# microsoft/SEAL-Embedded

Measured on AMD Instinct MI355X. Metric: CKKS ciphertexts/s (batched encode+encrypt), higher is better.
Workload: dtype u32; 1 GPU; C2: n=4096, 3x30-bit RNS primes, symmetric encode+encrypt, batch=65536 per GPU; n=4096, nprimes=3, mode=sym, batch_per_gpu=65536, global_batch=65536, parallelism=batch-sharded x1, bytes_per_unit=106624

## Files before the change

include/seal_embedded_amd.h:

```cpp
#ifndef SEAL_EMBEDDED_AMD_H
#define SEAL_EMBEDDED_AMD_H

#include <stdbool.h>
#include <stddef.h>
#include <stdint.h>
#include <sys/types.h>

#ifdef __cplusplus
typedef double _Complex se_complex;
#else
#include <complex.h>
typedef double complex se_complex;
#endif

#ifdef __cplusplus
extern "C" {
#endif

#define SE_SUCCESS 0
#define SE_ERR_NO_MEMORY -12
#define SE_ERR_INVALD_ARGUMENT -22
#define SE_ERR_UNKNOWN -1000
#define SE_ERR_MINIMUM -9999
#define SE_ERR_NO_DEVICE -19
// ... 175 lines not shown
int se_amd_write_ciphertext_text(const char *path, int append, const float *values, size_t vlen,
                                 const uint32_t *c0, const uint32_t *c1, size_t n, size_t np);
int se_amd_save_secret_key_file(const char *dir, size_t n, const uint8_t *sk_packed);
int se_amd_save_public_key_files(const char *dir, size_t n, size_t np, const uint32_t *q,
                                 const uint32_t *pk0, const uint32_t *pk1);

enum
{
    SE_AMD_STAGE_CBD = 0,
    SE_AMD_STAGE_UNIFORM = 1,
    SE_AMD_STAGE_TERNARY = 2,
    SE_AMD_STAGE_ENCODE_ENCRYPT = 3,
    SE_AMD_STAGE_ENCODE_RNS = 4,
    SE_AMD_STAGE_NTT_FUSE = 5,
    SE_AMD_STAGE_COUNT = 6
};
int se_amd_set_profiling(se_amd_ctx *ctx, int enabled);
int se_amd_stage_ms(se_amd_ctx *ctx, float *ms ,
                    uint64_t *launches , int reset);
int se_amd_host_tables(size_t degree, size_t nprimes, uint32_t *q, uint32_t *const_ratio,
                       double *scale, uint16_t *index_map, double *ifft_w, uint32_t *ntt_rw,
                       uint32_t *intt_rw);
int se_amd_ifft_table_sha256(se_amd_ctx *ctx, char out_hex[65]);
int se_amd_set_reject_list_capacity(se_amd_ctx *ctx, uint32_t cap);
int se_amd_set_speculation_capacity(se_amd_ctx *ctx, uint32_t cap);
int se_amd_set_host_chunk(se_amd_ctx *ctx, size_t ciphertexts);
int se_amd_reserve(se_amd_ctx *ctx, size_t B);
int se_amd_set_debug_flags(se_amd_ctx *ctx, uint32_t flags);
int se_amd_set_pipeline(se_amd_ctx *ctx, int overlap, int split);
int se_amd_set_asym_chunks(se_amd_ctx *ctx, size_t chunks);
const char *se_amd_last_error(void);
const char *se_amd_version(void);

#ifdef __cplusplus
}
#endif

#include "seal_embedded_amd_lower.h"

#endif
```

seal-embedded_amd/__init__.py:

```python
import ctypes as C
import os
import subprocess

HERE = os.path.dirname(os.path.abspath(__file__))
LIB_PATH = os.path.join(HERE, "lib", "libseal_embedded_amd.so")
CSRC = os.path.join(HERE, "csrc")
INCLUDE = os.path.join(os.path.dirname(HERE), "include", "seal_embedded_amd.h")

STAGES = ("cbd", "uniform", "ternary", "encode_encrypt", "encode_rns", "ntt_fuse")

SE_SUCCESS = 0


class SealEmbeddedAmdError(RuntimeError):
    pass


TESTHOOKS_LIB_DIR = os.path.join(HERE, "lib", "testhooks")


def build_library(jobs=8, verbose=False):
    cmd = ["make", "-C", CSRC, f"-j{jobs}", "all", "testhooks"]
    if not verbose:
        cmd.insert(1, "-s")
# ... 3 lines not shown

_lib = None

EXPORTED_SYMBOLS = (
    "se_setup_custom", "se_setup", "se_setup_default", "se_encrypt_seeded", "se_encrypt",
    "se_cleanup", "se_encrypt_batch",
    "se_amd_create", "se_amd_destroy", "se_amd_degree", "se_amd_nprimes", "se_amd_scale",
    "se_amd_moduli", "se_amd_index_map", "se_amd_set_secret_key", "se_amd_set_public_key",
    "se_amd_load_keys_from_dir", "se_amd_gen_public_key", "se_amd_gen_keys_batch", "se_amd_encrypt_sym_device", "se_amd_encrypt_asym_device", "se_amd_encrypt_sym_seeded_device",
    "se_amd_expand_c1_device",
    "se_amd_encode_ntt_device", "se_amd_encrypt_sym_host", "se_amd_encrypt_asym_host",
    "se_amd_encode_device", "se_amd_ntt_device", "se_amd_intt_device", "se_amd_decrypt_decode_device", "se_amd_prng_blocks_device",
    "se_amd_sample_uniform_device", "se_amd_sample_ternary_device", "se_amd_sample_cbd_device",
    "se_amd_pack_ternary_host", "se_amd_word_ops_device", "se_amd_pack_seal_ciphertext_host", "se_amd_format_poly_text",
    "se_amd_format_values_text", "se_amd_write_ciphertext_text", "se_amd_save_secret_key_file",
    "se_amd_save_public_key_files", "se_amd_set_profiling", "se_amd_stage_ms",
    "se_amd_group_create", "se_amd_group_destroy", "se_amd_group_size", "se_amd_group_ctx", "se_amd_group_device",
    "se_amd_group_partition", "se_amd_group_set_secret_key", "se_amd_group_set_public_key", "se_amd_group_reserve",
    "se_amd_encrypt_sym_multi_device", "se_amd_encrypt_asym_multi_device", "se_amd_encode_ntt_multi_device",
    "se_amd_set_reject_list_capacity", "se_amd_set_speculation_capacity", "se_amd_set_host_chunk", "se_amd_host_tables", "se_amd_ifft_table_sha256", "se_amd_reserve", "se_amd_set_debug_flags", "se_amd_set_pipeline", "se_amd_set_asym_chunks", "se_amd_last_error", "se_amd_version",
    "se_amd_set_secret_keyring", "se_amd_set_public_keyring", "se_amd_encrypt_sym_keyed_device",
    "se_amd_encrypt_asym_keyed_device", "se_amd_decrypt_decode_keyed_device",
    "se_amd_decrypt_full_device", "se_amd_decrypt_full_keyed_device", "se_amd_crt_constants",
)


def lib():
    global _lib
    if _lib is not None:
        return _lib
    if not os.path.exists(LIB_PATH):
        raise SealEmbeddedAmdError(
            f"{LIB_PATH} is missing: run __graft_entry__.build() (hipcc --offload-arch=gfx950). "
            "There is no CPU fallback.")
    L = C.CDLL(LIB_PATH)
    vp, sz, i32, u32 = C.c_void_p, C.c_size_t, C.c_int, C.c_uint32
    L.se_amd_last_error.restype = C.c_char_p
    L.se_amd_version.restype = C.c_char_p
    L.se_amd_create.argtypes = [C.POINTER(vp), sz, sz, i32]
    L.se_amd_destroy.argtypes = [vp]
    L.se_amd_destroy.restype = None
    L.se_amd_degree.argtypes = [vp]
    L.se_amd_degree.restype = sz
    L.se_amd_nprimes.argtypes = [vp]
    L.se_amd_nprimes.restype = sz
    L.se_amd_scale.argtypes = [vp]
# ... 19 lines not shown
    L.se_amd_prng_blocks_device.argtypes = [vp, vp, vp, vp, sz, sz, vp]
    L.se_amd_sample_uniform_device.argtypes = [vp, vp, vp, sz, vp, vp, vp]
    L.se_amd_sample_ternary_device.argtypes = [vp, vp, sz, vp, vp, vp]
    L.se_amd_sample_cbd_device.argtypes = [vp, vp, vp, sz, sz, vp, vp]
    L.se_amd_word_ops_device.argtypes = [vp, sz, i32, vp, vp, vp, vp, sz, vp]
    L.se_amd_pack_ternary_host.argtypes = [vp, sz, vp]
    L.se_amd_pack_ternary_host.restype = None
    L.se_amd_pack_seal_ciphertext_host.argtypes = [vp, vp, sz, sz, vp]
    L.se_amd_pack_seal_ciphertext_host.restype = None
    L.se_amd_format_poly_text.argtypes = [C.c_char_p, vp, sz, vp, sz]
    L.se_amd_format_poly_text.restype = sz
    L.se_amd_format_values_text.argtypes = [C.c_char_p, vp, sz, vp, sz]
    L.se_amd_format_values_text.restype = sz
    L.se_amd_write_ciphertext_text.argtypes = [C.c_char_p, i32, vp, sz, vp, vp, sz, sz]
    L.se_amd_save_secret_key_file.argtypes = [C.c_char_p, sz, vp]
    L.se_amd_save_public_key_files.argtypes = [C.c_char_p, sz, sz, vp, vp, vp]
    L.se_amd_set_profiling.argtypes = [vp, i32]
    L.se_amd_stage_ms.argtypes = [vp, vp, vp, i32]
    L.se_amd_set_reject_list_capacity.argtypes = [vp, u32]
    L.se_amd_set_speculation_capacity.argtypes = [vp, u32]
    L.se_amd_set_host_chunk.argtypes = [vp, sz]
    L.se_amd_host_tables.argtypes = [sz, sz, vp, vp, vp, vp, vp, vp, vp]
    L.se_amd_ifft_table_sha256.argtypes = [vp, C.c_char_p]
    L.se_amd_reserve.argtypes = [vp, sz]
    L.se_amd_set_debug_flags.argtypes = [vp, u32]
    L.se_amd_set_pipeline.argtypes = [vp, i32, i32]
    L.se_amd_set_asym_chunks.argtypes = [vp, sz]
    L.se_amd_set_secret_keyring.argtypes = [vp, sz, vp]
    L.se_amd_set_public_keyring.argtypes = [vp, sz, vp, vp]
    L.se_amd_encrypt_sym_keyed_device.argtypes = [vp, vp, sz, vp, vp, vp, vp, vp, vp, vp, vp, vp]
    L.se_amd_encrypt_asym_keyed_device.argtypes = [vp, vp, sz, vp, vp, vp, vp, vp, vp, vp, vp]
    L.se_amd_decrypt_decode_keyed_device.argtypes = [vp, vp, vp, sz, vp, sz, vp, vp, vp, vp]
    L.se_amd_decrypt_full_device.argtypes = [vp, vp, vp, sz, vp, vp, vp, vp, vp]
    L.se_amd_decrypt_full_keyed_device.argtypes = [vp, vp, vp, sz, vp, vp, vp, vp, vp, vp]
    L.se_amd_crt_constants.argtypes = [sz, sz, vp, vp]
    _lib = L
    return L


def _check(rc, what):
    if rc < 0:
        msg = lib().se_amd_last_error().decode(errors="replace")
        raise SealEmbeddedAmdError(f"{what} failed with code {rc}: {msg}")
    return rc


# ... 124 lines not shown
        except Exception:
            pass

    def scale(self):
        return float(self.L.se_amd_scale(self.h))

    def moduli(self):
        import numpy as np
        q = np.zeros(self.np, dtype=np.uint32)
        _check(self.L.se_amd_moduli(self.h, _ptr(q)), "se_amd_moduli")
        return [int(x) for x in q]

    def index_map(self):
        import numpy as np
        m = np.zeros(self.n, dtype=np.uint16)
        _check(self.L.se_amd_index_map(self.h, _ptr(m)), "se_amd_index_map")
        return m

    def ifft_table_sha256(self):
        buf = C.create_string_buffer(65)
        _check(self.L.se_amd_ifft_table_sha256(self.h, buf), "se_amd_ifft_table_sha256")
        return buf.value.decode()

    def set_secret_key(self, sk_packed):
        import numpy as np
        sk = np.ascontiguousarray(sk_packed, dtype=np.uint8)
        assert sk.size == self.n // 4
        _check(self.L.se_amd_set_secret_key(self.h, _ptr(sk)), "se_amd_set_secret_key")

    def set_public_key(self, pk0, pk1):
        import numpy as np
        pk0 = np.ascontiguousarray(pk0, dtype=np.uint32)
        pk1 = np.ascontiguousarray(pk1, dtype=np.uint32)
        assert pk0.size == self.np * self.n == pk1.size
        _check(self.L.se_amd_set_public_key(self.h, _ptr(pk0), _ptr(pk1)), "se_amd_set_public_key")

    def gen_public_key(self, sk_packed, pk_seed, ep_seed):
        import numpy as np
        sk = np.ascontiguousarray(sk_packed, dtype=np.uint8)
        s1 = np.frombuffer(bytes(pk_seed), dtype=np.uint8).copy()
        s2 = np.frombuffer(bytes(ep_seed), dtype=np.uint8).copy()
        pk0 = np.zeros((self.np, self.n), dtype=np.uint32)
        pk1 = np.zeros_like(pk0)
        _check(self.L.se_amd_gen_public_key(self.h, _ptr(sk), _ptr(s1), _ptr(s2), _ptr(pk0),
                                            _ptr(pk1)), "se_amd_gen_public_key")
        return pk0, pk1
# ... 227 lines not shown
```

seal-embedded_amd/csrc/kernels/encode_encrypt.hip:

```cpp
#include <hip/hip_runtime.h>

#include <algorithm>

#include "../se_types.h"
#include "kernel_args.h"
#include "transform.cuh"

namespace seamd {

__device__ __forceinline__ void load16(uint32_t (&v)[16], const uint32_t *p)
{
    const uint4 *p4 = reinterpret_cast<const uint4 *>(p);
#pragma unroll
    for (int i = 0; i < 4; i++)
    {
        uint4 w      = p4[i];
        v[4 * i]     = w.x;
        v[4 * i + 1] = w.y;
        v[4 * i + 2] = w.z;
        v[4 * i + 3] = w.w;
    }
}

__device__ __forceinline__ void store16(uint32_t *p, const uint32_t (&v)[16])
// ... 203 lines not shown
    }
    wg = __ockl_wgred_or_i32((ok ? 0 : kWgOverflow) | (small ? 0 : kWgNotSmall) | (nonfinite ? kWgNonfinite : 0));
    if constexpr (sizeof(MT) == 4)
    {
        small = !(wg & kWgNotSmall);
        if (status && t == 0 && small) status[b] = 1;
    }
    else
    {
        const bool declined = !BRANCH_EXACT && (wg & kWgNonfinite);
        if (status && t == 0 && !declined) status[b] = (wg & kWgOverflow) ? 0 : 1;
    }
}

template <int MODE>
constexpr int enc_quad_stride()
{
    return MODE == kModeAsym ? 28 : 20;
}

constexpr int kWgRisky          = 8;
constexpr double kHalfDelta     = 3.0e-14 * 1.001;
constexpr size_t kPairParkWords = 5120;

template <int LOGN, int MODE, bool GENERAL, bool PAIR, typename MT>
__device__ __forceinline__ void encrypt_tail(const DevParams &P, const DevTables &T, const EncArgs &A,
                                             const size_t b, unsigned char *smem, MT (&m)[16], const bool small)
{
    const int t = thread_index<GENERAL>();
    using G            = XformGeom<LOGN>;
    constexpr bool ASYM3 = LOGN <= 12;
    constexpr int N    = G::N;
    constexpr int CTOP = LOGN - 4;
    uint32_t *lds32 = reinterpret_cast<uint32_t *>(smem);

    const int np   = P.nprimes;

    if constexpr (MODE == kModeSym)
    {
#pragma unroll
        for (int e = 0; e < 16; e++) m[e] += A.err[b * N + (e << CTOP) + t];
    }
    else if constexpr (MODE == kModeAsym)
    {
#pragma unroll
        for (int e = 0; e < 16; e++) m[e] += A.err[b * 2 * N + (e << CTOP) + t];
// ... 121 lines not shown
                st_poly<QUADS>(A.c1 + pb, out, tg);
            }
            reduce_signed16(m, x, q, crh, crl, small);
            ntt_tiles<LOGN>(x, RW, q, lds32, t);
#pragma unroll
            for (int e = 0; e < 16; e++) x[e] = canon4(x[e], q, two_q);
            to_quads(x);
            if (A.ntt_pte) st_poly<QUADS>(A.ntt_pte + pb, x, tg);
            park_load();
            {
                uint32_t w[16], wp[16], out[16];
                ld_pairs<QUADS>(w, wp, T.pk0 + kb, tg);
#pragma unroll
                for (int e = 0; e < 16; e++)
                {
                    uint32_t pr = csub(mul_shoup_lazy(uh[e], w[e], wp[e], q), q);
                    out[e]      = csub(pr + x[e], q);
                }
                st_poly<QUADS>(A.c0 + pb, out, tg);
            }
        }
        else
        {
            uint32_t a_pre[16];
            if constexpr (MODE == kModeSym && QUADS) ld_poly<QUADS>(a_pre, A.c1 + pb, tg);
            reduce_signed16(m, x, q, crh, crl, small);
            ntt_tiles<LOGN>(x, RW, q, lds32, t);
            if constexpr (MODE != kModeSym)
            {
#pragma unroll
                for (int e = 0; e < 16; e++) x[e] = canon4(x[e], q, two_q);
            }
            to_quads(x);
            if (A.ntt_pte)
            {
                uint32_t cx[16];
#pragma unroll
                for (int e = 0; e < 16; e++) cx[e] = canon4(x[e], q, two_q);
                st_poly<QUADS>(A.ntt_pte + pb, cx, tg);
            }
            if constexpr (MODE == kModeSym)
            {
                uint32_t a[16], w[16], wp[16], out[16];
                if constexpr (QUADS)
                {
#pragma unroll
                    for (int e = 0; e < 16; e++) a[e] = a_pre[e];
                }
                else
                    ld_poly<QUADS>(a, A.c1 + pb, tg);
// ... 82 lines not shown
    for (int p = 0; p < 2; p++)
    {
        const float s = nf[p].x + nf[p].y;
        nonfinite[p]  = s != s;
    }
    __syncthreads();
    const float ss_all[2] = {(part[0] + part[2]) + (part[4] + part[6]), (part[1] + part[3]) + (part[5] + part[7])};
    double re[16], im[16];
    {
        const int Tl    = t & 127;
        const float *my = sv + (t >> 7) * (N / 2);
        const uint4 *mp = reinterpret_cast<const uint4 *>(T.gather_map);
        uint4 m0 = mp[Tl], m1 = mp[TH + Tl];
        uint32_t packed[8] = {m0.x, m0.y, m0.z, m0.w, m1.x, m1.y, m1.z, m1.w};
#pragma unroll
        for (int e = 0; e < 16; e++)
        {
            uint32_t idx = (packed[e >> 1] >> (16 * (e & 1))) & 0xFFFFu;
            re[e]        = (double)my[idx];
            im[e]        = 0.0;
        }
    }
    __syncthreads();
    ifft_pair_real_half<LOGN>(re, im, T.ifft_w, plane, t);

    int flags = 0;
#pragma unroll
    for (int p = 0; p < 2; p++)
    {
        const double delta = kHalfDelta * P.n_inv * sqrt(2.0 * (double)N * (double)ss_all[p]);
        double amax = 0.0;
        bool risky  = false;
#pragma unroll
        for (int e = 0; e < 16; e++)
        {
            const double x = e < 8 ? re[8 * p + e] : im[8 * p + e - 8];
            const double v = __dmul_rn(x, P.n_inv);
            const double a = fabs(v);
            const double g = __dsub_rn(a, trunc(a));
            risky          = risky || (fabs(__dsub_rn(g, 0.5)) < delta);
            const double r = round_half_away(v);
            amax           = fmax(amax, fabs(r));
            if (p == 0) mA[e] = (int32_t)r; else mB[e] = (int32_t)r;
        }
        const bool sm = amax < P.small_bound && !nonfinite[p];
        flags |= ((sm ? 0 : kWgNotSmall) | (nonfinite[p] ? kWgNonfinite : 0) | (risky ? kWgRisky : 0)) << (8 * p);
    }
// ... 736 lines not shown
    return hipGetLastError();
}

hipError_t launch_key_sanitize(const uint32_t *raw, uint32_t *idx, uint32_t *bad, size_t K, size_t B, hipStream_t st)
{
    if (B == 0) return hipSuccess;
    if (K == 0 || K > 0xFFFFFFFFull) return hipErrorInvalidValue;
    hipError_t e = hipMemsetAsync(bad, 0, sizeof(uint32_t), st);
    if (e != hipSuccess) return e;
    hipLaunchKernelGGL(k_key_sanitize, dim3((unsigned)((B + 255) / 256)), dim3(256), 0, st, raw, idx, bad,
                       (uint32_t)K, B);
    return hipGetLastError();
}

hipError_t launch_key_reject(const DevParams &P, const KeyRejectArgs &A, size_t B, hipStream_t st)
{
    if (B == 0) return hipSuccess;
    const unsigned grid = (unsigned)std::min<size_t>(B, (size_t)4 * (P.num_cus ? P.num_cus : 256u));
    hipLaunchKernelGGL(k_key_reject, dim3(grid), dim3(256), 0, st, A);
    return hipGetLastError();
}

template <int LOGN, int MODE>
static hipError_t launch_enc_mode(const DevParams &P, const DevTables &T, const EncArgs &A, size_t B,
                                  hipStream_t st, const KeyRing *ring)
{
    using G             = XformGeom<LOGN>;
    const size_t planes = (size_t)G::SLOTS * sizeof(double);
    const size_t quads  = (size_t)(G::N / 16) * enc_quad_stride<MODE>() * sizeof(uint32_t);
    size_t shmem_fast = planes, shmem_gen = planes;
    if (LOGN <= 12)
    {
        const size_t ntt_planes = (size_t)(MODE == kModeAsym ? 3 : 1) * G::SLOTS * sizeof(uint32_t);
        shmem_fast = MODE == kModeAsym ? std::max(planes, std::max(ntt_planes, quads)) : std::max(planes, ntt_planes + quads);
        shmem_gen  = MODE == kModeAsym ? std::max(planes, ntt_planes) : std::max(planes, ntt_planes + quads);
    }
    hipError_t e = hipMemsetAsync(A.general, 0, sizeof(uint32_t), st);
    if (e != hipSuccess) return e;
    EncArgs Af = A;
    Af.count   = B;
    if (enc_pairs<LOGN, MODE>()) shmem_fast = std::max(shmem_fast, (kPairParkWords + (size_t)G::N) * sizeof(uint32_t));
    const unsigned grid_fast = (unsigned)(enc_pairs<LOGN, MODE>() ? (B + 1) / 2 : B);
    const unsigned cus  = P.num_cus ? P.num_cus : 256u;
    const unsigned grid = (unsigned)std::min<size_t>(B, (size_t)4 * cus);
    if constexpr (MODE != kModeEncodeOnly)
    {
        if (ring)
        {
            (void)hipFuncSetAttribute((const void *)k_encode_encrypt_keyed<LOGN, MODE>,
                                      hipFuncAttributeMaxDynamicSharedMemorySize, (int)shmem_fast);
            hipLaunchKernelGGL((k_encode_encrypt_keyed<LOGN, MODE>), dim3(grid_fast), dim3(G::THREADS), shmem_fast, st,
                               P, T, Af, *ring);
            e = hipGetLastError();
            if (e != hipSuccess) return e;
            (void)hipFuncSetAttribute((const void *)k_encode_encrypt_general_keyed<LOGN, MODE>,
                                      hipFuncAttributeMaxDynamicSharedMemorySize, (int)shmem_gen);
            hipLaunchKernelGGL((k_encode_encrypt_general_keyed<LOGN, MODE>), dim3(grid), dim3(G::THREADS), shmem_gen,
                               st, P, T, A, *ring);
            return hipGetLastError();
        }
    }
    (void)hipFuncSetAttribute((const void *)k_encode_encrypt<LOGN, MODE>,
                              hipFuncAttributeMaxDynamicSharedMemorySize, (int)shmem_fast);
    hipLaunchKernelGGL((k_encode_encrypt<LOGN, MODE>), dim3(grid_fast), dim3(G::THREADS), shmem_fast, st, P, T,
// ... 13 lines not shown
{
    if (!A.general) return hipErrorInvalidValue;
    switch (mode)
    {
        case kModeSym: return launch_enc_mode<LOGN, kModeSym>(P, T, A, B, st, ring);
        case kModeAsym: return launch_enc_mode<LOGN, kModeAsym>(P, T, A, B, st, ring);
        default:
            if (ring) return hipErrorInvalidValue;
            return launch_enc_mode<LOGN, kModeEncodeOnly>(P, T, A, B, st, nullptr);
    }
}

hipError_t launch_encode_encrypt(const DevParams &P, const DevTables &T, const EncArgs &A, int mode,
                                 size_t B, hipStream_t st, const KeyRing *ring)
{
    if (B == 0) return hipSuccess;
    switch (P.logn)
    {
        case 10: return launch_enc<10>(P, T, A, mode, B, st, ring);
        case 11: return launch_enc<11>(P, T, A, mode, B, st, ring);
        case 12: return launch_enc<12>(P, T, A, mode, B, st, ring);
        case 13: return launch_enc<13>(P, T, A, mode, B, st, ring);
        case 14: return launch_enc<14>(P, T, A, mode, B, st, ring);
        default: return hipErrorInvalidValue;
    }
}

template <int LOGN, bool ADD_ERR>
static hipError_t launch_enc_rns_e(const DevParams &P, const DevTables &T, const EncArgs &A, size_t B,
                                   hipStream_t st)
{
    using G      = XformGeom<LOGN>;
    size_t shmem = (size_t)G::SLOTS * sizeof(double);
    if (!A.general) return hipErrorInvalidValue;
    hipError_t e = hipMemsetAsync(A.general, 0, sizeof(uint32_t), st);
    if (e != hipSuccess) return e;
    (void)hipFuncSetAttribute((const void *)k_encode_rns<LOGN, ADD_ERR>,
                              hipFuncAttributeMaxDynamicSharedMemorySize, (int)shmem);
    hipLaunchKernelGGL((k_encode_rns<LOGN, ADD_ERR>), dim3((unsigned)B), dim3(G::THREADS), shmem, st, P, T, A);
    e = hipGetLastError();
    if (e != hipSuccess) return e;
    const unsigned cus  = P.num_cus ? P.num_cus : 256u;
    const unsigned grid = (unsigned)std::min<size_t>(B, (size_t)cus);
    (void)hipFuncSetAttribute((const void *)k_encode_rns_general<LOGN, ADD_ERR>,
                              hipFuncAttributeMaxDynamicSharedMemorySize, (int)shmem);
    hipLaunchKernelGGL((k_encode_rns_general<LOGN, ADD_ERR>), dim3(grid), dim3(G::THREADS), shmem, st, P, T, A);
// ... 108 lines not shown
```

seal-embedded_amd/csrc/kernels/kernel_args.h:

```cpp
#pragma once
#include <hip/hip_runtime.h>
#include <stddef.h>
#include <stdint.h>

#include "../se_types.h"

namespace seamd {

struct EncArgs
{
    const float *values;
    const int8_t *err;
    const int8_t *ucodes;
    uint32_t *c0;
    uint32_t *c1;
    uint32_t *ntt_pte;
    int64_t *pte;
    uint8_t *status;
    uint32_t *general;
    uint8_t *compact;
    size_t count;
};
struct UniformArgs
{
// ... 28 lines not shown
};
struct TernaryArgs
{
    const uint8_t *seeds;
    int8_t *codes;
    uint64_t *ctr_out;
    uint32_t n;
    uint32_t B;
    const uint64_t *ctr_in;
    uint32_t num_cus;
    uint32_t debug_flags;
};

struct KeyRing
{
    const uint32_t *k0;
    const uint32_t *k1;
    const uint32_t *idx;
    size_t stride;
};

hipError_t launch_encode_encrypt(const DevParams &, const DevTables &, const EncArgs &, int mode,
                                 size_t B, hipStream_t, const KeyRing *ring = nullptr);
hipError_t launch_encode_rns(const DevParams &, const DevTables &, const EncArgs &, bool add_err,
                             size_t B, hipStream_t);
hipError_t launch_ntt_fuse(const DevParams &, const DevTables &, const EncArgs &, int mode, int j,
                           size_t B, hipStream_t, const KeyRing *ring = nullptr);
hipError_t launch_decrypt_decode(const DevParams &, const DevTables &, const uint32_t *c0,
                                 const uint32_t *c1, uint32_t in_primes, int j, uint32_t *dec_ntt,
                                 uint32_t *pt, float *values, size_t B, hipStream_t,
                                 const KeyRing *ring = nullptr);
struct FullArgs
{
    const uint32_t *c0;
    const uint32_t *c1;
    int64_t *pte;
    float *values;
    double *values_f64;
    uint8_t *status;
};
hipError_t launch_decrypt_full(const DevParams &, const DevTables &, const CrtParams &, const FullArgs &, size_t B,
                               hipStream_t, const KeyRing *ring = nullptr);
hipError_t launch_ring_secret_ntt(const DevParams &, const DevTables &, int j, const uint8_t *packed, uint32_t *ring,
                                  size_t K, hipStream_t);
hipError_t launch_ring_pairs(const DevParams &, const uint32_t *vals, uint32_t *pairs, size_t K, hipStream_t);
hipError_t launch_key_sanitize(const uint32_t *raw, uint32_t *idx, uint32_t *bad, size_t K, size_t B, hipStream_t);
// ... 85 lines not shown
```

seal-embedded_amd/csrc/kernels/transform.cuh:

```cuda
#pragma once
#include <hip/hip_runtime.h>
#include <stdint.h>

#include <type_traits>

#include "modarith.cuh"

namespace seamd {

template <int BEGIN, int END, typename F>
__device__ __forceinline__ void static_for(F &&f)
{
    if constexpr (BEGIN < END)
    {
        f(std::integral_constant<int, BEGIN>{});
        static_for<BEGIN + 1, END>(f);
    }
}

template <int C>
__device__ __forceinline__ int tile_index(int t, int e)
{
    return ((t >> C) << (C + 4)) | (e << C) | (t & ((1 << C) - 1));
}

template <int CA, int CB>
__host__ __device__ constexpr int lds_slot(int k)
{
    constexpr int lo = CA < CB ? CA : CB, hi = CA < CB ? CB : CA;
    if constexpr (hi <= 4)
        return k + (k >> 4);
    else if constexpr (lo >= 5)
        return k;
    else
        return k + ((k >> 5) << 1);
}

template <int LOGN>
struct XformGeom
{
    static constexpr int N       = 1 << LOGN;
    static constexpr int THREADS = N / 16;
    static constexpr int PASSES  = (LOGN + 3) / 4;
    static constexpr int SLOTS   = N + N / 16;
    static constexpr int ifft_c(int p) { return (4 * p < LOGN - 4) ? 4 * p : LOGN - 4; }
    static constexpr int ntt_c(int p) { return (LOGN - 4 - 4 * p > 0) ? LOGN - 4 - 4 * p : 0; }
};

template <int C_FROM, int C_TO, typename T>
__device__ __forceinline__ void redeal(T (&v)[16], T *lds, int t)
{
    T *wr = lds + lds_slot<C_FROM, C_TO>(tile_index<C_FROM>(t, 0));
    static_for<0, 16>([&](auto ec) {
        constexpr int e = decltype(ec)::value;
        wr[lds_slot<C_FROM, C_TO>(e << C_FROM)] = v[e];
    });
    __syncthreads();
    const T *rd = lds + lds_slot<C_FROM, C_TO>(tile_index<C_TO>(t, 0));
    static_for<0, 16>([&](auto ec) {
        constexpr int e = decltype(ec)::value;
        v[e] = rd[lds_slot<C_FROM, C_TO>(e << C_TO)];
    });
    __syncthreads();
}

template <int STRIDE>
__device__ __forceinline__ void tile_to_quads(uint32_t (&x)[16], uint32_t *lds_region, int t)
{
    static_assert(STRIDE % 4 == 0 && STRIDE >= 16, "rows stay 16-byte aligned");
    const int lane = t & 63;
// ... 57 lines not shown
        if (dev_isnan(d)) d = dev_copysign(0.0, d);
        recalc = true;
    }
    if (recalc)
    {
        const double inf = __longlong_as_double(0x7FF0000000000000ll);
        x = __dmul_rn(inf, __dsub_rn(__dmul_rn(a, c), __dmul_rn(b, d)));
        y = __dmul_rn(inf, __dadd_rn(__dmul_rn(a, d), __dmul_rn(b, c)));
    }
}

template <bool EXACT>
__device__ __forceinline__ void cmul_annexg(double a, double b, double c, double d, double &x, double &y)
{
    const double ac = __dmul_rn(a, c), bd = __dmul_rn(b, d), ad = __dmul_rn(a, d), bc = __dmul_rn(b, c);
    x = __dsub_rn(ac, bd);
    y = __dadd_rn(ad, bc);
    if constexpr (EXACT)
    {
        if (dev_isnan(x) && dev_isnan(y)) cmul_recover(a, b, c, d, ac, bd, ad, bc, x, y);
    }
}

template <int LOGN, int C, int B_LO, int B_HI, bool EXACT = false>
__device__ __forceinline__ void ifft_pass(double (&re)[16], double (&im)[16],
                                          const double *__restrict__ W, int t)
{
    constexpr int N = 1 << LOGN;
    const int thi   = (C + 4 >= LOGN) ? 0 : (t >> C);
    static_for<B_LO, B_HI>([&](auto bc) {
        constexpr int b      = decltype(bc)::value;
        constexpr int h      = N >> (C + b + 1);
        constexpr int groups = 1 << (3 - b);
        static_for<0, groups>([&](auto gc) {
            constexpr int g = decltype(gc)::value;
            const int idx   = (C == 0) ? N + ((8 >> b) - 1 + g) * (N / 16) + t : h + ((thi << (3 - b)) | g);
            const double2 w = *reinterpret_cast<const double2 *>(W + 2 * idx);
            static_for<0, (1 << b)>([&](auto rc) {
                constexpr int e0 = (g << (b + 1)) | decltype(rc)::value;
                constexpr int e1 = e0 | (1 << b);
                double ar = __dsub_rn(re[e0], re[e1]);
                double ai = __dsub_rn(im[e0], im[e1]);
                re[e0]    = __dadd_rn(re[e0], re[e1]);
                im[e0]    = __dadd_rn(im[e0], im[e1]);
                cmul_annexg<EXACT>(ar, ai, w.x, w.y, re[e1], im[e1]);
            });
        });
    });
}

template <int LOGN>
__device__ __forceinline__ void ifft_pass0_real(double (&re)[16], double (&im)[16],
                                                const double *__restrict__ W, int t)
{
    constexpr int N = 1 << LOGN;
    static_for<0, 4>([&](auto bc) {
        constexpr int b      = decltype(bc)::value;
        constexpr int groups = 1 << (3 - b);
        static_for<0, groups>([&](auto gc) {
// ... 38 lines not shown
    redeal<0, 4>(im, plane, t);
    ifft_pass<LOGN, 4, 0, 4, EXACT>(re, im, W, t);
    if constexpr (LOGN <= 12)
    {
        constexpr int C2 = G::ifft_c(2);
        redeal<4, C2>(re, plane, t);
        redeal<4, C2>(im, plane, t);
        ifft_pass<LOGN, C2, 8 - C2, 4, EXACT>(re, im, W, t);
    }
    else
    {
        redeal<4, 8>(re, plane, t);
        redeal<4, 8>(im, plane, t);
        ifft_pass<LOGN, 8, 0, 4, EXACT>(re, im, W, t);
        constexpr int C3 = G::ifft_c(3);
        redeal<8, C3>(re, plane, t);
        redeal<8, C3>(im, plane, t);
        ifft_pass<LOGN, C3, 12 - C3, 4, EXACT>(re, im, W, t);
    }
}

template <int LOGN>
__device__ __forceinline__ void ifft_pair_real_half(double (&re)[16], double (&im)[16], const double *__restrict__ W,
                                                    double *plane, int t)
{
    static_assert(LOGN == 12, "four waves: two per plaintext in the register passes");
    using G             = XformGeom<LOGN>;
    constexpr int N     = 1 << LOGN;
    constexpr int HALF  = G::SLOTS / 2;
    static_assert(lds_slot<0, 4>(N / 2 - 1) < HALF && lds_slot<4, 8>(N / 2 - 1) < HALF, "a plaintext's lower half fits its region");
    const int T   = t & 127;
    double *mine  = plane + (t >> 7) * HALF;
    ifft_pass0_real<LOGN>(re, im, W, T);
    auto exchange_0_4 = [&](double (&v)[16]) {
        double *wr = mine + lds_slot<0, 4>(tile_index<0>(T, 0));
        static_for<0, 16>([&](auto ec) {
            constexpr int e = decltype(ec)::value;
            wr[lds_slot<0, 4>(e << 0)] = v[e];
        });
        __syncthreads();
        const double *rd = mine + lds_slot<0, 4>(tile_index<4>(T, 0));
        static_for<0, 16>([&](auto ec) {
            constexpr int e = decltype(ec)::value;
            v[e] = rd[lds_slot<0, 4>(e << 4)];
        });
        __syncthreads();
    };
    exchange_0_4(re);
    exchange_0_4(im);
    ifft_pass<LOGN, 4, 0, 4>(re, im, W, T);
    auto exchange_4_8 = [&](double (&v)[16]) {
        double *wr = mine + lds_slot<4, 8>(tile_index<4>(T, 0));
        static_for<0, 16>([&](auto ec) {
            constexpr int e = decltype(ec)::value;
            wr[lds_slot<4, 8>(e << 4)] = v[e];
        });
        __syncthreads();
        const double *rd = plane + lds_slot<4, 8>(tile_index<8>(t, 0));
        static_for<0, 8>([&](auto ec) {
            constexpr int e = decltype(ec)::value;
            v[e]     = rd[lds_slot<4, 8>(e << 8)];
            v[8 + e] = rd[HALF + lds_slot<4, 8>(e << 8)];
        });
        __syncthreads();
    };
    exchange_4_8(re);
    exchange_4_8(im);
    static_for<0, 3>([&](auto bc) {
        constexpr int b = decltype(bc)::value;
        constexpr int h = N >> (8 + b + 1);
        static_for<0, (4 >> b)>([&](auto gc) {
            constexpr int g = decltype(gc)::value;
            const double2 w = *reinterpret_cast<const double2 *>(W + 2 * (h + g));
            static_for<0, (2 << b)>([&](auto rc) {
                constexpr int r  = decltype(rc)::value;
                constexpr int e0 = ((r >> b) << 3) | (g << (b + 1)) | (r & ((1 << b) - 1));
                constexpr int e1 = e0 | (1 << b);
                double ar = __dsub_rn(re[e0], re[e1]);
                double ai = __dsub_rn(im[e0], im[e1]);
                re[e0]    = __dadd_rn(re[e0], re[e1]);
                im[e0]    = __dadd_rn(im[e0], im[e1]);
                cmul_annexg<false>(ar, ai, w.x, w.y, re[e1], im[e1]);
            });
        });
    });
    const double w1y = W[3];
#pragma unroll
    for (int e = 0; e < 16; e++)
    {
        const double i2 = __dadd_rn(im[e], im[e]);
        im[e]           = -__dmul_rn(i2, w1y);
        re[e]           = __dadd_rn(re[e], re[e]);
    }
}

template <int LOGN, int C, int B_LO, int B_HI>
__device__ __forceinline__ void ntt_pass(uint32_t (&x)[16], const uint32_t *__restrict__ RW,
                                         uint32_t q, uint32_t two_q, int t)
{
    constexpr int N = 1 << LOGN;
    const int thi   = (C + 4 >= LOGN) ? 0 : (t >> C);
    static_for<0, B_HI - B_LO>([&](auto sc) {
        constexpr int b      = B_HI - 1 - decltype(sc)::value;
        constexpr int h      = N >> (C + b + 1);
        constexpr int groups = 1 << (3 - b);
        static_for<0, groups>([&](auto gc) {
            constexpr int g = decltype(gc)::value;
            const int idx   = (C == 0) ? N + ((8 >> b) - 1 + g) * (N / 16) + t : h + ((thi << (3 - b)) | g);
            const uint2 rw  = *reinterpret_cast<const uint2 *>(RW + 2 * idx);
            static_for<0, (1 << b)>([&](auto rc) {
                constexpr int e0 = (g << (b + 1)) | decltype(rc)::value;
                constexpr int e1 = e0 | (1 << b);
                ct_butterfly(x[e0], x[e1], rw.x, rw.y, q, two_q);
            });
        });
    });
}

template <int LOGN>
__device__ __forceinline__ void ntt_tiles(uint32_t (&x)[16], const uint32_t *__restrict__ RW,
                                          uint32_t q, uint32_t *lds, int t)
{
    using G              = XformGeom<LOGN>;
    const uint32_t two_q = q << 1;
    constexpr int C0     = LOGN - 4;
    constexpr int C1     = G::ntt_c(1);
    ntt_pass<LOGN, C0, 0, 4>(x, RW, q, two_q, t);
    redeal<C0, C1>(x, lds, t);
    ntt_pass<LOGN, C1, 0, 4>(x, RW, q, two_q, t);
    if constexpr (LOGN <= 12)
    {
        redeal<C1, 0>(x, lds, t);
        ntt_pass<LOGN, 0, 0, C1>(x, RW, q, two_q, t);
    }
    else
    {
        constexpr int C2 = G::ntt_c(2);
        redeal<C1, C2>(x, lds, t);
        ntt_pass<LOGN, C2, 0, 4>(x, RW, q, two_q, t);
        redeal<C2, 0>(x, lds, t);
        ntt_pass<LOGN, 0, 0, C2>(x, RW, q, two_q, t);
    }
}

template <int LOGN, int C_FROM, int C_TO>
__device__ __forceinline__ void redeal3(uint32_t (&a)[16], uint32_t (&b)[16], uint32_t (&c)[16],
                                        uint32_t *lds, int t)
{
    constexpr int SL = XformGeom<LOGN>::SLOTS;
    uint32_t *wr = lds + lds_slot<C_FROM, C_TO>(tile_index<C_FROM>(t, 0));
    static_for<0, 16>([&](auto ec) {
        constexpr int e = decltype(ec)::value;
        constexpr int s = lds_slot<C_FROM, C_TO>(e << C_FROM);
        wr[s] = a[e], wr[SL + s] = b[e], wr[2 * SL + s] = c[e];
    });
    __syncthreads();
    const uint32_t *rd = lds + lds_slot<C_FROM, C_TO>(tile_index<C_TO>(t, 0));
    static_for<0, 16>([&](auto ec) {
        constexpr int e = decltype(ec)::value;
        constexpr int s = lds_slot<C_FROM, C_TO>(e << C_TO);
        a[e] = rd[s], b[e] = rd[SL + s], c[e] = rd[2 * SL + s];
    });
    __syncthreads();
}

template <int LOGN, int C, int B_LO, int B_HI>
__device__ __forceinline__ void ntt_pass3(uint32_t (&x)[16], uint32_t (&y)[16], uint32_t (&z)[16],
// ... 160 lines not shown
```

seal-embedded_amd/csrc/se_api.cpp:

```cpp
#include <errno.h>
#include <math.h>
#include <stdio.h>
#include <stdlib.h>
#include <string.h>
#include <sys/random.h>

#include <mutex>
#include <string>
#include <thread>
#include <vector>

#include "../../include/seal_embedded_amd.h"
#include "se_context.h"
#include "se_hostpipe.h"
#include "se_sha256.h"

namespace seamd {
const std::string &last_error();
}
using seamd::Context;
using seamd::HostPipe;

static_assert(seamd::kErrInvalid == SE_ERR_INVALD_ARGUMENT && seamd::kErrNoDevice == SE_ERR_NO_DEVICE &&
                  seamd::kErrHip == SE_ERR_HIP && seamd::kErrNoKey == SE_ERR_NO_KEY,
// ... 355 lines not shown
    if (!ctx) return SE_ERR_INVALD_ARGUMENT;
    ctx->c.rej_cap = cap;
    return SE_SUCCESS;
}

int se_amd_set_debug_flags(se_amd_ctx *ctx, uint32_t flags)
{
    if (!ctx) return SE_ERR_INVALD_ARGUMENT;
    ctx->c.debug_flags = flags;
    return SE_SUCCESS;
}

int se_amd_ifft_table_sha256(se_amd_ctx *ctx, char out_hex[65])
{
    if (!ctx || !out_hex) return SE_ERR_INVALD_ARGUMENT;
    const size_t n = ctx->c.hp.n;
    std::vector<double> w(2 * n);
    SEAMD_HIP(hipSetDevice(ctx->c.device));
    SEAMD_HIP(hipMemcpy(w.data(), ctx->c.dt.ifft_w, 2 * n * sizeof(double), hipMemcpyDeviceToHost));
    seamd::Sha256 h;
    h.update(w.data(), 2 * n * sizeof(double));
    const std::string hex = h.hex();
    memcpy(out_hex, hex.c_str(), 65);
    return SE_SUCCESS;
}

int se_amd_host_tables(size_t degree, size_t nprimes, uint32_t *q, uint32_t *const_ratio,
                       double *scale, uint16_t *index_map, double *ifft_w, uint32_t *ntt_rw,
                       uint32_t *intt_rw)
{
    seamd::HostParams hp;
    if (seamd::host_params_init(hp, degree, nprimes) != 0)
    {
        seamd::set_last_error("unsupported parameter set (degree, nprimes)");
        return SE_ERR_INVALD_ARGUMENT;
    }
    const size_t n = hp.n;
    for (size_t j = 0; j < hp.nprimes; j++)
    {
        if (q) q[j] = hp.q[j];
        if (const_ratio) const_ratio[2 * j] = hp.cr_lo[j], const_ratio[2 * j + 1] = hp.cr_hi[j];
    }
    if (scale) *scale = hp.scale;
    if (index_map)
    {
        std::vector<uint16_t> map, inv;
// ... 429 lines not shown
```

Before: 7.713 million ciphertexts/s.

## Stage middle-pass IFFT and NTT twiddle rows in LDS for paired kernel

Result: no change. 7.768 million ciphertexts/s (median of 3 runs) (+0.7%).

```diff
diff --git a/include/seal_embedded_amd.h b/include/seal_embedded_amd.h
--- a/include/seal_embedded_amd.h
+++ b/include/seal_embedded_amd.h
@@ -221,6 +221,7 @@
                        double *scale, uint16_t *index_map, double *ifft_w, uint32_t *ntt_rw,
                        uint32_t *intt_rw);
 int se_amd_ifft_table_sha256(se_amd_ctx *ctx, char out_hex[65]);
+int se_amd_fused_kernel_occupancy(se_amd_ctx *ctx, int mode, int keyed, int *workgroups_per_cu, size_t *lds_bytes);
 int se_amd_set_reject_list_capacity(se_amd_ctx *ctx, uint32_t cap);
 int se_amd_set_speculation_capacity(se_amd_ctx *ctx, uint32_t cap);
 int se_amd_set_host_chunk(se_amd_ctx *ctx, size_t ciphertexts);
diff --git a/seal-embedded_amd/__init__.py b/seal-embedded_amd/__init__.py
--- a/seal-embedded_amd/__init__.py
+++ b/seal-embedded_amd/__init__.py
@@ -49,6 +49,7 @@
     "se_amd_set_secret_keyring", "se_amd_set_public_keyring", "se_amd_encrypt_sym_keyed_device",
     "se_amd_encrypt_asym_keyed_device", "se_amd_decrypt_decode_keyed_device",
     "se_amd_decrypt_full_device", "se_amd_decrypt_full_keyed_device", "se_amd_crt_constants",
+    "se_amd_fused_kernel_occupancy",
 )
 
 
@@ -114,6 +115,7 @@
     L.se_amd_set_host_chunk.argtypes = [vp, sz]
     L.se_amd_host_tables.argtypes = [sz, sz, vp, vp, vp, vp, vp, vp, vp]
     L.se_amd_ifft_table_sha256.argtypes = [vp, C.c_char_p]
+    L.se_amd_fused_kernel_occupancy.argtypes = [vp, i32, i32, C.POINTER(i32), C.POINTER(sz)]
     L.se_amd_reserve.argtypes = [vp, sz]
     L.se_amd_set_debug_flags.argtypes = [vp, u32]
     L.se_amd_set_pipeline.argtypes = [vp, i32, i32]
@@ -284,6 +286,12 @@
         _check(self.L.se_amd_ifft_table_sha256(self.h, buf), "se_amd_ifft_table_sha256")
         return buf.value.decode()
 
+    def fused_kernel_occupancy(self, mode, keyed=False):
+        blocks, lds = C.c_int(0), C.c_size_t(0)
+        _check(self.L.se_amd_fused_kernel_occupancy(self.h, mode, int(keyed), C.byref(blocks), C.byref(lds)),
+               "se_amd_fused_kernel_occupancy")
+        return blocks.value, lds.value
+
     def set_secret_key(self, sk_packed):
         import numpy as np
         sk = np.ascontiguousarray(sk_packed, dtype=np.uint8)
diff --git a/seal-embedded_amd/csrc/kernels/encode_encrypt.hip b/seal-embedded_amd/csrc/kernels/encode_encrypt.hip
--- a/seal-embedded_amd/csrc/kernels/encode_encrypt.hip
+++ b/seal-embedded_amd/csrc/kernels/encode_encrypt.hip
@@ -249,6 +249,13 @@
 constexpr int kWgRisky          = 8;
 constexpr double kHalfDelta     = 3.0e-14 * 1.001;
 constexpr size_t kPairParkWords = 5120;
+constexpr size_t kPairIfftRowsWords = kPairParkWords + 4096;
+constexpr size_t kPairNttRowsWords  = kPairIfftRowsWords + root_rows<11, 4>() * (sizeof(double2) / 4);
+constexpr size_t kPairLdsWords      = kPairNttRowsWords + root_rows<12, 4>() * (sizeof(uint2) / 4);
+static_assert(kPairIfftRowsWords >= kPairParkWords + 16 * XformGeom<12>::THREADS, "the rows begin past the parked plaintext");
+static_assert(kPairIfftRowsWords >= (size_t)XformGeom<12>::SLOTS * 2, "the rows begin past the encoders' FP64 plane");
+static_assert(kPairIfftRowsWords % 4 == 0 && kPairNttRowsWords % 2 == 0, "16-byte twiddles, 8-byte root pairs");
+static_assert(kPairLdsWords * 4 <= 40960, "four workgroups per CU: 160 KiB / 4");
 
 template <int LOGN, int MODE, bool GENERAL, bool PAIR, typename MT>
 __device__ __forceinline__ void encrypt_tail(const DevParams &P, const DevTables &T, const EncArgs &A,
@@ -416,10 +423,16 @@
         }
         else
         {
+            const int ti = PAIR ? opaque_index(t) : 0;
+            uint2 rows_pre = {0u, 0u};
+            if constexpr (PAIR) rows_pre = ntt_rows_fetch<LOGN>(RW, ti);
             uint32_t a_pre[16];
             if constexpr (MODE == kModeSym && QUADS) ld_poly<QUADS>(a_pre, A.c1 + pb, tg);
             reduce_signed16(m, x, q, crh, crl, small);
-            ntt_tiles<LOGN>(x, RW, q, lds32, t);
+            if constexpr (PAIR)
+                ntt_tiles_rows<LOGN>(x, RW, q, lds32, t, reinterpret_cast<uint2 *>(lds32 + kPairNttRowsWords), ti, rows_pre);
+            else
+                ntt_tiles<LOGN>(x, RW, q, lds32, t);
             if constexpr (MODE != kModeSym)
             {
 #pragma unroll
@@ -548,7 +561,8 @@
         }
     }
     __syncthreads();
-    ifft_pair_real_half<LOGN>(re, im, T.ifft_w, plane, t);
+    ifft_pair_real_half<LOGN>(re, im, T.ifft_w, plane,
+                              reinterpret_cast<double2 *>(reinterpret_cast<uint32_t *>(smem) + kPairIfftRowsWords), t);
 
     int flags = 0;
 #pragma unroll
@@ -1331,8 +1345,7 @@
 }
 
 template <int LOGN, int MODE>
-static hipError_t launch_enc_mode(const DevParams &P, const DevTables &T, const EncArgs &A, size_t B,
-                                  hipStream_t st, const KeyRing *ring)
+static size_t enc_lds_bytes(bool general)
 {
     using G             = XformGeom<LOGN>;
     const size_t planes = (size_t)G::SLOTS * sizeof(double);
@@ -1344,11 +1357,20 @@
         shmem_fast = MODE == kModeAsym ? std::max(planes, std::max(ntt_planes, quads)) : std::max(planes, ntt_planes + quads);
         shmem_gen  = MODE == kModeAsym ? std::max(planes, ntt_planes) : std::max(planes, ntt_planes + quads);
     }
+    if (enc_pairs<LOGN, MODE>()) shmem_fast = std::max(shmem_fast, kPairLdsWords * sizeof(uint32_t));
+    return general ? shmem_gen : shmem_fast;
+}
+
+template <int LOGN, int MODE>
+static hipError_t launch_enc_mode(const DevParams &P, const DevTables &T, const EncArgs &A, size_t B,
+                                  hipStream_t st, const KeyRing *ring)
+{
+    using G                 = XformGeom<LOGN>;
+    const size_t shmem_fast = enc_lds_bytes<LOGN, MODE>(false), shmem_gen = enc_lds_bytes<LOGN, MODE>(true);
     hipError_t e = hipMemsetAsync(A.general, 0, sizeof(uint32_t), st);
     if (e != hipSuccess) return e;
     EncArgs Af = A;
     Af.count   = B;
-    if (enc_pairs<LOGN, MODE>()) shmem_fast = std::max(shmem_fast, (kPairParkWords + (size_t)G::N) * sizeof(uint32_t));
     const unsigned grid_fast = (unsigned)(enc_pairs<LOGN, MODE>() ? (B + 1) / 2 : B);
     const unsigned cus  = P.num_cus ? P.num_cus : 256u;
     const unsigned grid = (unsigned)std::min<size_t>(B, (size_t)4 * cus);
@@ -1408,6 +1430,49 @@
         case 12: return launch_enc<12>(P, T, A, mode, B, st, ring);
         case 13: return launch_enc<13>(P, T, A, mode, B, st, ring);
         case 14: return launch_enc<14>(P, T, A, mode, B, st, ring);
+        default: return hipErrorInvalidValue;
+    }
+}
+
+template <int LOGN, int MODE>
+static hipError_t enc_occupancy(bool keyed, int *blocks, size_t *lds_bytes)
+{
+    const size_t shmem = enc_lds_bytes<LOGN, MODE>(false);
+    const void *fn     = (const void *)k_encode_encrypt<LOGN, MODE>;
+    if constexpr (MODE != kModeEncodeOnly)
+    {
+        if (keyed) fn = (const void *)k_encode_encrypt_keyed<LOGN, MODE>;
+    }
+    else if (keyed)
+        return hipErrorInvalidValue;
+    hipError_t e = hipFuncSetAttribute(fn, hipFuncAttributeMaxDynamicSharedMemorySize, (int)shmem);
+    if (e != hipSuccess) return e;
+    if (lds_bytes) *lds_bytes = shmem;
+    return hipOccupancyMaxActiveBlocksPerMultiprocessor(blocks, fn, XformGeom<LOGN>::THREADS, shmem);
+}
+
+template <int LOGN>
+static hipError_t enc_occupancy_n(int mode, bool keyed, int *blocks, size_t *lds_bytes)
+{
+    switch (mode)
+    {
+        case kModeSym: return enc_occupancy<LOGN, kModeSym>(keyed, blocks, lds_bytes);
+        case kModeAsym: return enc_occupancy<LOGN, kModeAsym>(keyed, blocks, lds_bytes);
+        case kModeEncodeOnly: return enc_occupancy<LOGN, kModeEncodeOnly>(keyed, blocks, lds_bytes);
+        default: return hipErrorInvalidValue;
+    }
+}
+
+hipError_t encode_encrypt_occupancy(int logn, int mode, bool keyed, int *blocks, size_t *lds_bytes)
+{
+    if (!blocks) return hipErrorInvalidValue;
+    switch (logn)
+    {
+        case 10: return enc_occupancy_n<10>(mode, keyed, blocks, lds_bytes);
+        case 11: return enc_occupancy_n<11>(mode, keyed, blocks, lds_bytes);
+        case 12: return enc_occupancy_n<12>(mode, keyed, blocks, lds_bytes);
+        case 13: return enc_occupancy_n<13>(mode, keyed, blocks, lds_bytes);
+        case 14: return enc_occupancy_n<14>(mode, keyed, blocks, lds_bytes);
         default: return hipErrorInvalidValue;
     }
 }
diff --git a/seal-embedded_amd/csrc/kernels/kernel_args.h b/seal-embedded_amd/csrc/kernels/kernel_args.h
--- a/seal-embedded_amd/csrc/kernels/kernel_args.h
+++ b/seal-embedded_amd/csrc/kernels/kernel_args.h
@@ -74,6 +74,7 @@
 
 hipError_t launch_encode_encrypt(const DevParams &, const DevTables &, const EncArgs &, int mode,
                                  size_t B, hipStream_t, const KeyRing *ring = nullptr);
+hipError_t encode_encrypt_occupancy(int logn, int mode, bool keyed, int *blocks, size_t *lds_bytes);
 hipError_t launch_encode_rns(const DevParams &, const DevTables &, const EncArgs &, bool add_err,
                              size_t B, hipStream_t);
 hipError_t launch_ntt_fuse(const DevParams &, const DevTables &, const EncArgs &, int mode, int j,
diff --git a/seal-embedded_amd/csrc/kernels/transform.cuh b/seal-embedded_amd/csrc/kernels/transform.cuh
--- a/seal-embedded_amd/csrc/kernels/transform.cuh
+++ b/seal-embedded_amd/csrc/kernels/transform.cuh
@@ -46,6 +46,21 @@
     static constexpr int ifft_c(int p) { return (4 * p < LOGN - 4) ? 4 * p : LOGN - 4; }
     static constexpr int ntt_c(int p) { return (LOGN - 4 - 4 * p > 0) ? LOGN - 4 - 4 * p : 0; }
 };
+
+constexpr int kRootRow = 15;
+__host__ __device__ constexpr int root_row_col(int b, int g) { return 16 - (16 >> b) + g; }
+template <int LOGN, int C>
+__host__ __device__ constexpr int root_rows()
+{
+    return ((1 << LOGN) / 16 >> C) * kRootRow;
+}
+template <int LOGN, int C>
+__device__ __forceinline__ int root_row_source(int i)
+{
+    const int row = i / kRootRow, col = i - row * kRootRow;
+    const int b   = (col >= 8) + (col >= 12) + (col >= 14);
+    return (((1 << LOGN) >> (C + 1)) >> b) + (row << (3 - b)) + (col - root_row_col(b, 0));
+}
 
 template <int C_FROM, int C_TO, typename T>
 __device__ __forceinline__ void redeal(T (&v)[16], T *lds, int t)
@@ -149,11 +164,12 @@
     }
 }
 
-template <int LOGN, int C, int B_LO, int B_HI, bool EXACT = false>
+template <int LOGN, int C, int B_LO, int B_HI, bool EXACT = false, bool ROWS = false>
 __device__ __forceinline__ void ifft_pass(double (&re)[16], double (&im)[16],
                                           const double *__restrict__ W, int t)
 {
     constexpr int N = 1 << LOGN;
+    static_assert(!ROWS || (C > 0 && C + 4 < LOGN && B_LO == 0 && B_HI == 4), "rows hold a middle pass's four stages");
     const int thi   = (C + 4 >= LOGN) ? 0 : (t >> C);
     static_for<B_LO, B_HI>([&](auto bc) {
         constexpr int b      = decltype(bc)::value;
@@ -161,7 +177,8 @@
         constexpr int groups = 1 << (3 - b);
         static_for<0, groups>([&](auto gc) {
             constexpr int g = decltype(gc)::value;
-            const int idx   = (C == 0) ? N + ((8 >> b) - 1 + g) * (N / 16) + t : h + ((thi << (3 - b)) | g);
+            const int idx   = ROWS ? root_row_col(b, g)
+                              : (C == 0) ? N + ((8 >> b) - 1 + g) * (N / 16) + t : h + ((thi << (3 - b)) | g);
             const double2 w = *reinterpret_cast<const double2 *>(W + 2 * idx);
             static_for<0, (1 << b)>([&](auto rc) {
                 constexpr int e0 = (g << (b + 1)) | decltype(rc)::value;
@@ -246,7 +263,7 @@
 
 template <int LOGN>
 __device__ __forceinline__ void ifft_pair_real_half(double (&re)[16], double (&im)[16], const double *__restrict__ W,
-                                                    double *plane, int t)
+                                                    double *plane, double2 *rows, int t)
 {
     static_assert(LOGN == 12, "four waves: two per plaintext in the register passes");
     using G             = XformGeom<LOGN>;
@@ -255,7 +272,11 @@
     static_assert(lds_slot<0, 4>(N / 2 - 1) < HALF && lds_slot<4, 8>(N / 2 - 1) < HALF, "a plaintext's lower half fits its region");
     const int T   = t & 127;
     double *mine  = plane + (t >> 7) * HALF;
+    constexpr int ROWS = root_rows<LOGN - 1, 4>();
+    double2 staged     = {0.0, 0.0};
+    if (t < ROWS) staged = *reinterpret_cast<const double2 *>(W + 2 * root_row_source<LOGN, 4>(t));
     ifft_pass0_real<LOGN>(re, im, W, T);
+    if (t < ROWS) rows[t] = staged;
     auto exchange_0_4 = [&](double (&v)[16]) {
         double *wr = mine + lds_slot<0, 4>(tile_index<0>(T, 0));
         static_for<0, 16>([&](auto ec) {
@@ -272,7 +293,7 @@
     };
     exchange_0_4(re);
     exchange_0_4(im);
-    ifft_pass<LOGN, 4, 0, 4>(re, im, W, T);
+    ifft_pass<LOGN, 4, 0, 4, false, true>(re, im, reinterpret_cast<const double *>(rows + (T >> 4) * kRootRow), T);
     auto exchange_4_8 = [&](double (&v)[16]) {
         double *wr = mine + lds_slot<4, 8>(tile_index<4>(T, 0));
         static_for<0, 16>([&](auto ec) {
@@ -318,11 +339,12 @@
     }
 }
 
-template <int LOGN, int C, int B_LO, int B_HI>
+template <int LOGN, int C, int B_LO, int B_HI, bool ROWS = false>
 __device__ __forceinline__ void ntt_pass(uint32_t (&x)[16], const uint32_t *__restrict__ RW,
                                          uint32_t q, uint32_t two_q, int t)
 {
     constexpr int N = 1 << LOGN;
+    static_assert(!ROWS || (C > 0 && C + 4 < LOGN && B_LO == 0 && B_HI == 4), "rows hold a middle pass's four stages");
     const int thi   = (C + 4 >= LOGN) ? 0 : (t >> C);
     static_for<0, B_HI - B_LO>([&](auto sc) {
         constexpr int b      = B_HI - 1 - decltype(sc)::value;
@@ -330,7 +352,8 @@
         constexpr int groups = 1 << (3 - b);
         static_for<0, groups>([&](auto gc) {
             constexpr int g = decltype(gc)::value;
-            const int idx   = (C == 0) ? N + ((8 >> b) - 1 + g) * (N / 16) + t : h + ((thi << (3 - b)) | g);
+            const int idx   = ROWS ? root_row_col(b, g)
+                              : (C == 0) ? N + ((8 >> b) - 1 + g) * (N / 16) + t : h + ((thi << (3 - b)) | g);
             const uint2 rw  = *reinterpret_cast<const uint2 *>(RW + 2 * idx);
             static_for<0, (1 << b)>([&](auto rc) {
                 constexpr int e0 = (g << (b + 1)) | decltype(rc)::value;
@@ -367,6 +390,28 @@
     }
 }
 
+template <int LOGN>
+__device__ __forceinline__ uint2 ntt_rows_fetch(const uint32_t *__restrict__ RW, int i)
+{
+    uint2 rw = {0u, 0u};
+    if (i < root_rows<LOGN, 4>()) rw = *reinterpret_cast<const uint2 *>(RW + 2 * root_row_source<LOGN, 4>(i));
+    return rw;
+}
+
+template <int LOGN>
+__device__ __forceinline__ void ntt_tiles_rows(uint32_t (&x)[16], const uint32_t *__restrict__ RW, uint32_t q,
+                                               uint32_t *lds, int t, uint2 *rows, int i, uint2 staged)
+{
+    static_assert(LOGN == 12, "three passes: windows 8, 4, 0");
+    const uint32_t two_q = q << 1;
+    ntt_pass<LOGN, 8, 0, 4>(x, RW, q, two_q, t);
+    if (i < root_rows<LOGN, 4>()) rows[i] = staged;
+    redeal<8, 4>(x, lds, t);
+    ntt_pass<LOGN, 4, 0, 4, true>(x, reinterpret_cast<const uint32_t *>(rows + (t >> 4) * kRootRow), q, two_q, t);
+    redeal<4, 0>(x, lds, t);
+    ntt_pass<LOGN, 0, 0, 4>(x, RW, q, two_q, t);
+}
+
 template <int LOGN, int C_FROM, int C_TO>
 __device__ __forceinline__ void redeal3(uint32_t (&a)[16], uint32_t (&b)[16], uint32_t (&c)[16],
                                         uint32_t *lds, int t)
diff --git a/seal-embedded_amd/csrc/se_api.cpp b/seal-embedded_amd/csrc/se_api.cpp
--- a/seal-embedded_amd/csrc/se_api.cpp
+++ b/seal-embedded_amd/csrc/se_api.cpp
@@ -401,6 +401,14 @@
     h.update(w.data(), 2 * n * sizeof(double));
     const std::string hex = h.hex();
     memcpy(out_hex, hex.c_str(), 65);
+    return SE_SUCCESS;
+}
+
+int se_amd_fused_kernel_occupancy(se_amd_ctx *ctx, int mode, int keyed, int *workgroups_per_cu, size_t *lds_bytes)
+{
+    if (!ctx || !workgroups_per_cu) return SE_ERR_INVALD_ARGUMENT;
+    SEAMD_HIP(hipSetDevice(ctx->c.device));
+    SEAMD_HIP(seamd::encode_encrypt_occupancy((int)ctx->c.dp.logn, mode, keyed != 0, workgroups_per_cu, lds_bytes));
     return SE_SUCCESS;
 }
 
```
